# raymondfdavey/Conditioned-Diffusion-Models-UAD

Measured on AMD Instinct MI355X. Metric: reconstructed 128x128 slices/sec @ T=1000, higher is better.
Workload: dtype f32_emulated_f16x3

## Files before the change

conditioned-diffusion-models-uad_amd/_lib.py:

```python
from __future__ import annotations

import ctypes as C
import os

_HERE = os.path.dirname(os.path.abspath(__file__))
LIB_PATH = os.environ.get("CDDPM_LIB") or os.path.join(_HERE, "csrc", "libcddpm_hip.so")

CDDPM_MAX_LEVELS = 8


class UnetDesc(C.Structure):
    _fields_ = [
        ("in_channels", C.c_int32),
        ("out_channels", C.c_int32),
        ("model_channels", C.c_int32),
        ("num_levels", C.c_int32),
        ("channel_mult", C.c_int32 * CDDPM_MAX_LEVELS),
        ("num_res_blocks", C.c_int32),
        ("num_attention_resolutions", C.c_int32),
        ("attention_resolutions", C.c_int32 * CDDPM_MAX_LEVELS),
        ("head_channels", C.c_int32),
        ("cond_dim", C.c_int32),
        ("timesteps", C.c_int32),
        ("max_batch", C.c_int32),
# ... 42 lines not shown
    "cddpm_get_attention_family": (_i, [_vp]),
    "cddpm_set_precision": (_i, [_vp, _i]),
    "cddpm_get_precision": (_i, [_vp]),
    "cddpm_slice_status": (_i, [_vp, _fp, _i, _i, _i, _fp, _vp]),
    "cddpm_set_profiling": (_i, [_vp, _i]),
    "cddpm_get_profile": (_i, [_vp, _i, C.POINTER(C.c_double), C.POINTER(C.c_double), C.POINTER(C.c_double),
                               C.POINTER(_i64)]),
    "cddpm_num_blocks": (_i, [_vp]),
    "cddpm_block_name": (C.c_char_p, [_vp, _i]),
    "cddpm_set_tap": (_i, [_vp, _i, _fp]),
    "cddpm_block_shape": (_i, [_vp, _i, _i, _i, C.POINTER(_i), C.POINTER(_i), C.POINTER(_i)]),
    "cddpm_op_conv": (_i, [_vp, _fp, _i, _fp, _i, _fp, _i, _i, _fp, _fp, _i, _i, _fp, _i, _fp, _i, _i, _i, _vp]),
    "cddpm_op_conv_skip": (_i, [_vp, _fp, _i, _fp, _i, _fp, _fp, _i, _fp, _i, _fp, _fp, _i, _i, _i, _vp]),
    "cddpm_op_conv_gn": (_i, [_vp, _fp, _i, _fp, _fp, _i, _fp, _fp, _fp, _fp, _i, _i, _i, _vp]),
    "cddpm_op_gn_coef": (_i, [_vp, _fp, _i, _fp, _i, _fp, _fp, _fp, _fp, _i, _i, _vp]),
    "cddpm_op_attention": (_i, [_vp, _fp, _fp, _i, _i, _i, _vp]),
    "cddpm_op_attention_p16": (_i, [_vp, _fp, _fp, _i, _i, _i, _vp]),
    "cddpm_op_attention_h3": (_i, [_vp, _fp, _fp, _i, _i, _i, _vp]),
    "cddpm_encoder_create": (_i, [C.POINTER(_vp), _i, _i, _i, _i, _i]),
    "cddpm_encoder_destroy": (None, [_vp]),
    "cddpm_encoder_last_error": (C.c_char_p, [_vp]),
    "cddpm_encoder_num_weights": (_i, []),
    "cddpm_encoder_load_weights": (_i, [_vp, C.POINTER(C.c_char_p), C.POINTER(_fp), C.POINTER(_i64), _i]),
    "cddpm_encoder_forward": (_i, [_vp, _fp, _fp, _i, _i, _i, _vp]),
    "cddpm_op_conv_dgrad": (_i, [_vp, _fp, _i, _fp, _i, _i, _fp, _i, _i, _i, _vp]),
    "cddpm_op_conv_wgrad": (_i, [_vp, _fp, _i, _fp, _i, _fp, _i, _i, _fp, _i, _i, _fp, _fp, _i, _i, _i, _vp]),
    "cddpm_op_bias_grad": (_i, [_vp, _fp, _i64, _i, _fp, _vp]),
    "cddpm_op_attention_backward": (_i, [_vp, _fp, _fp, _fp, _i, _i, _i, _vp]),
    "cddpm_op_attention_backward_p16": (_i, [_vp, _fp, _fp, _fp, _i, _i, _i, _vp]),
    "cddpm_op_attention_backward_h3": (_i, [_vp, _fp, _fp, _fp, _i, _i, _i, _vp]),
    "cddpm_op_linear_backward": (_i, [_vp, _fp, _fp, _fp, _i, _i, _i, _i, _fp, _fp, _fp, _vp]),
    "cddpm_op_linear": (_i, [_vp, _fp, _fp, _fp, _i, _i, _i, _i, _fp, _vp]),
    "cddpm_op_conv_in1": (_i, [_vp, _fp, _fp, _fp, _fp, _i, _i, _i, _i, _vp]),
    "cddpm_op_head": (_i, [_vp, _fp, _fp, _fp, C.c_float, _fp, _fp, _i, _i, _i, _i, _vp]),
    "cddpm_op_pool_act": (_i, [_vp, _fp, _fp, _fp, _fp, _i, _i, _i, _i, _vp]),
    "cddpm_op_unpool2": (_i, [_vp, _fp, _fp, _i, _i, _i, _i, C.c_float, _i, _vp]),
    "cddpm_op_sumpool2": (_i, [_vp, _fp, _fp, _i, _i, _i, _i, _i, _vp]),
    "cddpm_op_add_inplace": (_i, [_vp, _fp, _fp, _i64, _vp]),
    "cddpm_op_act_dropout": (_i, [_vp, _fp, _fp, _i, _fp, _u64, _u32, _u64, _u32, C.c_double, _i, _i, _i, _vp]),
    "cddpm_op_dropout_scale": (_i, [_vp, _fp, _u64, _u32, _u64, _u32, C.c_double, _i, _i, _i, _vp]),
    "cddpm_op_chan_image_corr": (_i, [_vp, _fp, _fp, _i, _fp, _i, _fp, _i, _i, _i, _i, _vp]),
    "cddpm_op_head_dgrad": (_i, [_vp, _fp, _fp, _fp, _i, _i, _i, _i, _vp]),
    "cddpm_op_loss": (_i, [_vp, _fp, _fp, _fp, _i, _i, _i, C.c_float, _fp, _fp, _vp]),
    "cddpm_op_loss_box": (_i, [_vp, _fp, _fp, _fp, _vp, _fp, _i, _i, _i, _i, _i, _i, C.c_float, _vp, _fp, _fp, _vp]),
    "cddpm_box_q_sample": (_i, [_vp, _fp, _fp, _vp, _i, _fp, _fp, _i, _vp, _fp, _i, _i, _i, _i, _vp]),
    "cddpm_box_stitch": (_i, [_vp, _fp, _vp, _vp, _i, _fp, _i, _i, _i, _i, _vp]),
    "cddpm_op_adam": (_i, [_vp, _fp, _fp, _fp, _fp, _i64, C.c_float, C.c_float, C.c_float, C.c_float, _i, C.c_float, _vp]),
    "cddpm_set_train_precision": (_i, [_i]),
    "cddpm_get_train_precision": (_i, []),
    "cddpm_op_grad_check": (_i, [_vp, _fp, _i64, _vp, _vp]),
    "cddpm_op_guard_commit": (_i, [_vp, _vp, C.c_float, C.c_float, _vp]),
    "cddpm_op_adam_guarded": (_i, [_vp, _fp, _fp, _fp, _fp, _i64, C.c_float, C.c_float, C.c_float, C.c_float, C.c_float, _vp, _vp]),
    "cddpm_op_loss_scaled": (_i, [_vp, _fp, _fp, _fp, _i, _i, _i, _vp, _fp, _fp, _vp]),
    "cddpm_op_adam_scaled": (_i, [_vp, _fp, _fp, _fp, _fp, _i64, C.c_float, C.c_float, C.c_float, C.c_float, C.c_float, _vp, _vp, _vp]),
    "cddpm_op_scaler_update": (_i, [_vp, _vp, _vp, C.c_float, C.c_float, _i, _vp]),
    "cddpm_op_gn_silu_backward": (_i, [_vp, _fp, _fp, _i, _fp, _fp, _fp, _fp, _i, _fp, _fp, _fp, _fp, _fp, _fp, _i, _fp, _i, _i, _i, _vp]),
    "cddpm_op_enc_pack_w": (_i, [_vp, _fp, _i, _i, _i, _fp, _fp, _vp]),
    "cddpm_op_enc_conv": (_i, [_vp, _fp, _fp, _fp, _i, _i, _i, _i, _i, _i, _i, _i, _vp]),
    "cddpm_op_enc_conv_wgrad": (_i, [_vp, _fp, _fp, _fp, _i, _i, _i, _i, _i, _i, _i, _vp]),
    "cddpm_op_enc_pack_w_p16": (_i, [_vp, _fp, _i, _i, _i, _vp, _vp, _vp]),
    "cddpm_op_enc_conv_p16": (_i, [_vp, _fp, _vp, _fp, _i, _i, _i, _i, _i, _i, _i, _i, _vp]),
    "cddpm_op_enc_conv_wgrad_p16": (_i, [_vp, _fp, _fp, _fp, _i, _i, _i, _i, _i, _i, _i, _vp]),
    "cddpm_op_enc_stem": (_i, [_vp, _fp, _fp, _fp, _i, _i, _i, _vp]),
    "cddpm_op_enc_stem_wgrad": (_i, [_vp, _fp, _fp, _fp, _i, _i, _i, _vp]),
    "cddpm_op_enc_bn_forward": (_i, [_vp, _fp, _fp, _fp, _fp, _fp, _i, C.c_float, C.c_float, _fp, _fp, _fp, _fp, _i64, _i, _i, _vp]),
    "cddpm_op_enc_bn_backward": (_i, [_vp, _fp, _fp, _fp, _fp, _fp, _fp, _i, _fp, _fp, _fp, _fp, _i64, _i, _i, _vp]),
# ... 88 lines not shown
```

conditioned-diffusion-models-uad_amd/csrc/cddpm_api.hip:

```cpp
#include "cddpm_ctx.h"

#include <cmath>
#include <cstdarg>
#include <cstdio>
#include <cstdlib>

using namespace cddpm;

namespace {
thread_local std::string g_create_error;
}

int cddpm::fail(cddpm_ctx* h, const char* fmt, ...) {
    char buf[1024];
    va_list ap;
    va_start(ap, fmt);
    vsnprintf(buf, sizeof buf, fmt, ap);
    va_end(ap);
    if (h) h->err = buf; else g_create_error = buf;
    return -1;
}

namespace {

// ... 252 lines not shown
        if (op.kind != OP_HEAD) maxact = std::max(maxact, elems);
        if (op.push) {
            float* p = nullptr;
            want(&p, elems);
            h->hs.push_back(p);
        }
    }
    for (const ResW& r : h->res) maxC = std::max(maxC, (size_t)std::max(r.Cin, r.Cout));
    for (const AttnW& a : h->attn) maxC = std::max(maxC, (size_t)a.C);
    want(&h->bufA, maxact);
    want(&h->bufB, maxact);
    want(&h->bufH, maxact);
    want(&h->bufP0, maxact / 4 + 16);
    want(&h->bufP1, maxact / 4 + 16);
    size_t maxqkv = 0, maxatt = 0;
    for (const Op& op : h->prog)
        if (op.kind == OP_ATTN) {
            const BlockInfo& bi = h->blocks[op.block];
            const AttnW& a = h->attn[op.idx];
            int dsa = bi.ds;
            for (const Op& o2 : h->prog)
                if (o2.block == op.block && o2.kind == OP_RES && h->res[o2.idx].up) dsa = bi.ds * 2;
            const size_t n = HW / ((size_t)dsa * dsa);
            maxqkv = std::max(maxqkv, B * n * 3 * a.C);
            maxatt = std::max(maxatt, B * n * a.C);
        }
    want(&h->qkvbuf, maxqkv);
    want(&h->attbuf, maxatt);
    want(&h->headP, B * HW * 9);
    want(&h->model_out, B * HW);
    {
        auto nrec_at = [&](int ds) {
            const int hh = d.max_h / ds, ww = d.max_w / ds;
            return std::max(std::max(conv_stat_records(hh, ww), conv_stat_records_up2(hh, ww)), gn_nsplit(1, hh * ww));
        };
        size_t pi = 0;
        for (const Op& op : h->prog)
            if (op.push) {
                const BlockInfo& bi = h->blocks[op.block];
                const size_t cap = B * (size_t)nrec_at(bi.ds) * bi.C * 2;
                float* sp = nullptr;
                want(&sp, cap);
                if (do_alloc) h->stat[h->hs[pi]] = {sp, cap, STAT_NONE};
                ++pi;
            }
        size_t maxrc = 0;
        for (const BlockInfo& bi : h->blocks) maxrc = std::max(maxrc, (size_t)nrec_at(bi.ds) * bi.C);
        float* work[3] = {h->bufA, h->bufB, h->bufH};
        for (int i = 0; i < 3; ++i) {
            float* sp = nullptr;
            want(&sp, B * maxrc * 2);
            if (do_alloc) h->stat[work[i]] = {sp, B * maxrc * 2, STAT_NONE};
        }
    }
    want(&h->coef, 3 * B * maxC);
    want(&h->kpart, (size_t)KSPLIT_PLANE_FLOATS);
    const size_t rows = std::max<size_t>(d.timesteps, B);
    want(&h->tab, (size_t)d.timesteps * h->sumE);
    want(&h->cpart, B * (size_t)h->sumE);
    want(&h->scratch0, rows * std::max(h->half, d.model_channels));
    want(&h->scratch1, rows * h->half);
    for (int i = 0; i < 5; ++i) want(&h->sched[i], d.timesteps);
    want(&h->qs_sa, d.timesteps);
    want(&h->qs_s1, d.timesteps);
    total += B * sizeof(int);
    if (do_alloc && *rc == 0) *rc = dev_alloc(h, &h->d_t, B);
    for (const WeightSpec& w : h->wspecs) total += (size_t)w.numel * sizeof(float);
// ... 140 lines not shown
        return fail(h, "H=%d W=%d invalid for this handle (multiples of %d, max %dx%d)", H, W, q > 4 ? q : 4, h->d.max_h, h->d.max_w);
    if (h->cond_B != B) return fail(h, "cddpm_prepare_cond was last called for B=%d, this call has B=%d", h->cond_B, B);
    return 0;
}

int stage_t(cddpm_ctx* h, const int32_t* t_dev, int t_uniform, int B, hipStream_t s) {
    if (t_dev) {
        launch_copy_clamp_int(h->d_t, t_dev, B, 0, h->d.timesteps - 1, s);
    } else {
        if (t_uniform < 0 || t_uniform >= h->d.timesteps) return fail(h, "t=%d outside [0, %d)", t_uniform, h->d.timesteps);
        launch_fill_int(h->d_t, B, t_uniform, s);
    }
    return 0;
}

int forward_impl(cddpm_ctx* h, const float* x, float* out, int B, int H, int W, hipStream_t s) {
    for (auto& kv : h->stat) kv.second.valid_count = STAT_NONE;
    h->cur_H = H; h->cur_W = W;
    std::vector<int> stack;
    int npush = 0;
    const float* cur = nullptr;
    int curC = 0, curds = 1;
    float* pp[2] = {h->bufA, h->bufB};
    int ppi = 0;
    for (size_t oi = 0; oi < h->prog.size(); ++oi) {
        const Op& op = h->prog[oi];
        const BlockInfo& bi = h->blocks[op.block];
        float* dst;
        if (op.push) dst = h->hs[npush];
        else { dst = pp[ppi]; ppi ^= 1; }
        const int Hc = H / curds, Wc = W / curds;
        switch (op.kind) {
            case OP_IN: {
                Prof pi(h, PC_OTHER, 18.0 * B * H * W * h->d.model_channels, 4.0 * B * (double)H * W * (h->d.model_channels + 1), s);
                launch_conv_in1(x, h->in_w, h->in_b, dst, B, H, W, h->d.model_channels, s);
            }
                curC = h->d.model_channels;
                break;
            case OP_RES: {
                const ResW& r = h->res[op.idx];
                const float* x1 = nullptr;
                int C1 = 0;
                if (op.concat) {
                    const int si = stack.back();
                    stack.pop_back();
                    x1 = h->hs[si];
                    C1 = r.Cin - curC;
                }
                if (dst == cur) { dst = pp[ppi]; ppi ^= 1; }
                if (run_res(h, r, cur, curC, x1, C1, dst, B, Hc, Wc, s)) return -1;
                curC = r.Cout;
                if (r.down) curds *= 2;
                if (r.up) curds /= 2;
                break;
            }
            case OP_ATTN:
                if (dst == cur) { dst = pp[ppi]; ppi ^= 1; }
                if (run_attn(h, h->attn[op.idx], cur, dst, B, Hc, Wc, s)) return -1;
                break;
            case OP_HEAD: {
                if (gn_coef(h, cur, curC, nullptr, 0, B, H * W, h->out_norm, false, 0, s)) return -1;
                Prof ph(h, PC_OTHER, 18.0 * B * H * W * curC, 4.0 * B * (double)H * W * (curC + 19), s);
                launch_head_dots(cur, h->coef, h->head_w9, h->headP, B, H * W, curC, s);
                launch_head_gather(h->headP, h->head_bias, nullptr, out, B, H, W, s);
                dst = nullptr;
                break;
            }
        }
// ... 722 lines not shown
```

conditioned-diffusion-models-uad_amd/csrc/cddpm_ops.hip:

```cpp
#include "cddpm_ctx.h"

#include <cmath>

using namespace cddpm;

template <class Request> static size_t counted(Request&& request) {
    OpScratch sc;
    request(sc);
    return sc.off;
}

extern "C" {

int cddpm_op_set_scratch(cddpm_handle h, size_t bytes) {
    if (!h) return -1;
    HIPCHECK(h, hipSetDevice(h->device));
    HIPCHECK(h, hipDeviceSynchronize());
    if (h->arena) { (void)hipFree(h->arena); h->arena = nullptr; h->arena_bytes = 0; }
    if (bytes) { HIPCHECK(h, hipMalloc(&h->arena, bytes)); h->arena_bytes = bytes; }
    return 0;
}

static int need_zero_bias(cddpm_ctx* h) {
    if (h->zero_bias) return 0;
// ... 292 lines not shown
    OP_EPILOGUE()
}

static float* linear_backward_scratch(OpScratch& sc, int M, int N, int K, int silu_in) {
    const size_t nscr = linear_backward_scratch_floats(M, N, K, silu_in);
    return nscr ? sc.n<float>(nscr) : nullptr;
}
size_t cddpm_op_linear_backward_scratch(int M, int N, int K, int silu_in) {
    return counted([&](OpScratch& sc) { linear_backward_scratch(sc, M, N, K, silu_in); });
}
int cddpm_op_linear_backward(cddpm_handle h, const float* x_dev, const float* w_dev, const float* dy_dev, int M, int N, int K,
                             int silu_in, float* dw_dev, float* db_dev, float* dx_dev, void* stream) {
    OP_PROLOGUE(PC_OTHER, 0.0, 0.0, M >= 1 && N >= 1 && K >= 1 && x_dev && w_dev && dy_dev && dw_dev, "cddpm_op_linear_backward: bad arguments")
    OpScratch sc(h, s);
    float* a = linear_backward_scratch(sc, M, N, K, silu_in);
    SCRATCH_CHECK(sc)
    launch_linear_backward(x_dev, w_dev, dy_dev, M, N, K, silu_in, a, dw_dev, db_dev, dx_dev, s);
    OP_EPILOGUE()
}

int cddpm_op_linear(cddpm_handle h, const float* x_dev, const float* w_dev, const float* b_dev, int M, int N, int K, int silu_in,
                    float* y_dev, void* stream) {
    OP_CHECK(M >= 1 && N >= 1 && K >= 1 && K % 4 == 0, "cddpm_op_linear: unsupported shape (M %d, N %d, K %d: all >= 1, K a multiple of 4)", M, N, K)
    OP_PROLOGUE(PC_OTHER, 0.0, 0.0, x_dev && w_dev && y_dev && !(((uintptr_t)x_dev | (uintptr_t)w_dev) & 15),
                "cddpm_op_linear: NULL argument, or x_dev / w_dev not 16-byte aligned")
    launch_linear(x_dev, K, w_dev, K, 0, b_dev, y_dev, N, M, N, K, silu_in, s);
    OP_EPILOGUE()
}
int cddpm_op_conv_in1(cddpm_handle h, const float* x_dev, const float* w_dev, const float* b_dev, float* out_dev, int B, int H, int W,
                      int C, void* stream) {
    OP_CHECK(B >= 1 && H >= 1 && W >= 1 && (long long)B * H * W < (1ll << 31) && C >= 64 && C % 64 == 0 && C <= 512,
             "cddpm_op_conv_in1: unsupported shape (B %d, H %d, W %d: all >= 1, B * H * W < 2^31; C %d: a multiple of 64, at most 512)", B, H, W, C)
    OP_PROLOGUE(PC_OTHER, 0.0, 0.0, x_dev && w_dev && b_dev && out_dev, "cddpm_op_conv_in1: NULL argument")
    launch_conv_in1(x_dev, w_dev, b_dev, out_dev, B, H, W, C, s);
    OP_EPILOGUE()
}
static float* head_scratch(OpScratch& sc, int B, int H, int W) { return sc.n<float>((size_t)B * H * W * 9); }
size_t cddpm_op_head_scratch(int B, int H, int W, int) { return counted([&](OpScratch& sc) { head_scratch(sc, B, H, W); }); }
int cddpm_op_head(cddpm_handle h, const float* x_dev, const float* coef_dev, const float* w9_dev, float bias, const float* bias_dev,
                  float* out_dev, int B, int H, int W, int C, void* stream) {
    static_assert(head_dots_lds_bytes(head_max_channels()) <= LDS_BYTES_PER_WORKGROUP && head_dots_lds_bytes(head_max_channels() + 32) > LDS_BYTES_PER_WORKGROUP,
                  "the widest head");
    OP_CHECK(B >= 1 && H >= 1 && W >= 1 && C >= 32 && C % 32 == 0 && C <= head_max_channels(),
             "cddpm_op_head: unsupported shape (B %d, H %d, W %d: all >= 1; C %d: a multiple of 32, at most %d)", B, H, W, C, head_max_channels())
    OP_PROLOGUE(PC_OTHER, 0.0, 0.0, x_dev && coef_dev && w9_dev && out_dev, "cddpm_op_head: NULL argument")
    OpScratch sc(h, s);
    float* P = head_scratch(sc, B, H, W);
    SCRATCH_CHECK(sc)
    launch_head_dots(x_dev, coef_dev, w9_dev, P, B, H * W, C, s);
    launch_head_gather(P, bias, bias_dev, out_dev, B, H, W, s);
    OP_EPILOGUE()
}
static bool resample_shape_ok(int B, int H, int W, int C) { return B >= 1 && H >= 2 && W >= 2 && H % 2 == 0 && W % 2 == 0 && C >= 4 && C % 4 == 0; }
int cddpm_op_pool_act(cddpm_handle h, const float* x_dev, const float* coef_dev, float* hp_dev, float* xp_dev, int B, int H, int W, int C,
                      void* stream) {
    OP_CHECK(resample_shape_ok(B, H, W, C), "cddpm_op_pool_act: unsupported shape (B %d >= 1; H %d, W %d: even, >= 2; C %d: a multiple of 4, >= 4)", B, H, W, C)
    OP_PROLOGUE(PC_OTHER, 0.0, 0.0, x_dev && coef_dev && hp_dev && xp_dev, "cddpm_op_pool_act: NULL argument")
    launch_pool_act(x_dev, coef_dev, hp_dev, xp_dev, B, H, W, C, s);
    OP_EPILOGUE()
}
int cddpm_op_unpool2(cddpm_handle h, const float* dyp_dev, float* dx_dev, int B, int H, int W, int C, float scale, int accumulate, void* stream) {
    OP_CHECK(resample_shape_ok(B, H, W, C), "cddpm_op_unpool2: unsupported shape (B %d >= 1; H %d, W %d: even, >= 2; C %d: a multiple of 4, >= 4)", B, H, W, C)
    OP_PROLOGUE(PC_OTHER, 0.0, 0.0, dyp_dev && dx_dev, "cddpm_op_unpool2: NULL argument")
    launch_unpool2(dyp_dev, dx_dev, B, H, W, C, scale, accumulate, s);
    OP_EPILOGUE()
}
int cddpm_op_sumpool2(cddpm_handle h, const float* dy_dev, float* dxp_dev, int B, int H, int W, int C, int accumulate, void* stream) {
// ... 600 lines not shown
```

conditioned-diffusion-models-uad_amd/csrc/conv_split.h:

```cpp
#pragma once
#include <hip/hip_runtime.h>

namespace cddpm {

typedef float f32x16 __attribute__((ext_vector_type(16)));
typedef float v4f __attribute__((ext_vector_type(4)));
typedef float v2f __attribute__((ext_vector_type(2)));
typedef __bf16 bf16x8 __attribute__((ext_vector_type(8)));
typedef __bf16 bf16x4 __attribute__((ext_vector_type(4)));
typedef _Float16 f16x8 __attribute__((ext_vector_type(8)));
typedef _Float16 f16x4 __attribute__((ext_vector_type(4)));

template <int NS> struct SplitT;
template <> struct SplitT<3> {
    typedef bf16x8 v8; typedef bf16x4 v4;
    static __device__ __forceinline__ f32x16 mfma(v8 a, v8 b, f32x16 c) { return __builtin_amdgcn_mfma_f32_32x32x16_bf16(a, b, c, 0, 0, 0); }
};
template <> struct SplitT<2> {
    typedef f16x8 v8; typedef f16x4 v4;
    static __device__ __forceinline__ f32x16 mfma(v8 a, v8 b, f32x16 c) { return __builtin_amdgcn_mfma_f32_32x32x16_f16(a, b, c, 0, 0, 0); }
};

__device__ __forceinline__ float silu_x6(float v) {
    const float t = fminf(-v * 1.44269502162933349609375f, 126.0f);
    float tl = __builtin_fmaf(-v, 1.44269502162933349609375f, -t);
    tl = __builtin_fmaf(-v, 1.925963033500011e-08f, tl);
    tl = (t < 126.0f) ? tl : 0.0f;
    float e = __builtin_amdgcn_exp2f(t);
    e = __builtin_fmaf(e, tl * 0.693147180559945f, e);
    return v * __builtin_amdgcn_rcpf(1.0f + e);
}

__device__ __forceinline__ v4f silu_x6_v4(const v4f v) {
    const v4f nl2e = {-1.44269502162933349609375f, -1.44269502162933349609375f, -1.44269502162933349609375f, -1.44269502162933349609375f};
    const v4f nl2e_lo = {-1.925963033500011e-08f, -1.925963033500011e-08f, -1.925963033500011e-08f, -1.925963033500011e-08f};
    const v4f lim = {126.0f, 126.0f, 126.0f, 126.0f};
    const v4f ln2 = {0.693147180559945f, 0.693147180559945f, 0.693147180559945f, 0.693147180559945f};
    const v4f one = {1.0f, 1.0f, 1.0f, 1.0f};
    const v4f t = __builtin_elementwise_min(v * nl2e, lim);
    v4f tl = __builtin_elementwise_fma(v, nl2e, -t);
    tl = __builtin_elementwise_fma(v, nl2e_lo, tl);
    v4f e = {__builtin_amdgcn_exp2f(t.x), __builtin_amdgcn_exp2f(t.y), __builtin_amdgcn_exp2f(t.z), __builtin_amdgcn_exp2f(t.w)};
    e = __builtin_elementwise_fma(e, tl * ln2, e);
    const v4f d = one + e;
    const v4f r = {__builtin_amdgcn_rcpf(d.x), __builtin_amdgcn_rcpf(d.y), __builtin_amdgcn_rcpf(d.z), __builtin_amdgcn_rcpf(d.w)};
    return v * r;
}

template <int NS>
__device__ __forceinline__ void split_x4(const v4f v, typename SplitT<NS>::v4 (&t)[NS]) {
    typedef typename SplitT<NS>::v4 q4;
    v4f r = v;
#pragma unroll
    for (int s = 0; s < NS; ++s) {
        t[s] = __builtin_convertvector(r, q4);
        r = r - __builtin_convertvector(t[s], v4f);
    }
}

}
```

conditioned-diffusion-models-uad_amd/csrc/conv_x6.hip:

```cpp
#include "kernels.h"
#include "conv_split.h"
#include <algorithm>
#include <cstdlib>
#include <cstring>
#include <type_traits>
#include <vector>

namespace cddpm {

static constexpr int ROWS = 8;
template <int TAPS, int NS, bool HI1 = false, int NB = 1>
__global__ __launch_bounds__(64 * ROWS) void conv_split_kernel(const ConvArgs a) {
    static_assert(NB == 1 || (NB == 2 && NS == 2 && TAPS != 1), "two cout blocks per workgroup: 16 x 16 fp16 form, LDS-DMA loop (3x3 and folded 2x2) only");
    typedef typename SplitT<NS>::v8 frag;
    constexpr int SP = 4 * NS;
    constexpr int THREADS = 64 * ROWS;
    constexpr bool UP2 = (TAPS == 4);
    constexpr int PAD = (TAPS == 9) ? 1 : 0;
    constexpr int PW = UP2 ? 33 : 32 + 2 * PAD;
    constexpr int PH = UP2 ? ROWS + 1 : ROWS + 2 * PAD;
    constexpr int NPIX = PW * PH;
    constexpr int NK = (NPIX * 8 + THREADS - 1) / THREADS;
    constexpr int FOLD = (TAPS == 9) ? 3 : (TAPS == 4 ? 2 : 1);
    constexpr int WSLOTS = 128 * SP;
// ... 78 lines not shown
    const bool have_coef = (a.coef != nullptr);

    auto wslab = [&](int chunk, int tap) -> const v4f* {
        if (chunk >= nch) { chunk = 0; tap = 0; }
        return (chunk < nch_main) ? (wmain + ((size_t)chunk * TAPS + tap) * WSLOTS)
                                  : (wskip + (size_t)(chunk - nch_main) * WSLOTS);
    };
    auto load_act = [&](int chunk) {
        const float* base;
        int Cs, c0;
        const bool main_seg = chunk < nch_main;
        if (main_seg) {
            const int ch = chunk << 5;
            if (ch < a.C0) { base = a.src0; Cs = a.C0; c0 = ch; }
            else           { base = a.src1; Cs = a.C1; c0 = ch - a.C0; }
        } else {
            const int ch = (chunk - nch_main) << 5;
            if (ch < a.S0) { base = a.skip0; Cs = a.S0; c0 = ch; }
            else           { base = a.skip1; Cs = a.S1; c0 = ch - a.S0; }
        }
        const float* ubase = base + ((size_t)b * a.srcH * a.srcW * Cs + c0);
#pragma unroll
        for (int k = 0; k < NK; ++k) {
            const int p = (main_seg || ((centre >> k) & 1u)) ? psrc[k] : -1;
            v4f v = v4f{0.f, 0.f, 0.f, 0.f};
            if (p >= 0) v = *reinterpret_cast<const v4f*>(ubase + (__umul24((unsigned)p, (unsigned)Cs) + 4u * (unsigned)c4));
            areg[k] = v;
        }
    };
    typename SplitT<NS>::v4 sreg[NK][NS];
    auto transform_act = [&](int chunk) {
        const bool main_seg = chunk < nch_main;
        const bool do_silu = main_seg && a.silu;
        v4f cm = v4f{0.f, 0.f, 0.f, 0.f}, ca = v4f{1.f, 1.f, 1.f, 1.f}, cd = cm;
        const bool aff = main_seg && have_coef;
        if (aff) {
            const int ci = (chunk << 3) + c4;
            cm = ldsC[ci];
            ca = ldsC[(Cin >> 2) + ci];
            cd = ldsC[2 * (Cin >> 2) + ci];
        }
#pragma unroll
        for (int k = 0; k < NK; ++k) {
            v4f v = areg[k];
            const int p = (main_seg || ((centre >> k) & 1u)) ? psrc[k] : -1;
            if (p >= 0) {
                v = (v - cm) * ca + cd;
                if (do_silu) {
                    if constexpr (NS == 2) v = silu_x6_v4(v);
                    else { v.x = silu_x6(v.x); v.y = silu_x6(v.y); v.z = silu_x6(v.z); v.w = silu_x6(v.w); }
                }
            }
            split_x4<NS>(v, sreg[k]);
        }
    };
    auto write_act = [&]() {
        v2f* dst = reinterpret_cast<v2f*>(ldsA);
#pragma unroll
        for (int k = 0; k < NK; ++k) {
            const int q = (tid >> 3) + (THREADS / 8) * k;
            if (q < NPIX) {
#pragma unroll
                for (int sp = 0; sp < (HI1 ? 1 : NS); ++sp) {
                    const int sl = M16 ? (q * 8 + ((4 * sp + (c4 >> 1)) ^ (int)((colswz >> (3 * k)) & 7u))) : slot_a(q, sp, c4 >> 1);
                    dst[sl * 2 + (c4 & 1)] = __builtin_bit_cast(v2f, sreg[k][sp]);
                }
            }
        }
    };
    auto store_act = [&](int chunk) { transform_act(chunk); write_act(); };

    typedef float f32x4 __attribute__((ext_vector_type(4)));
    f32x16 acc[2][2], tot[2][2];
    f32x4 acc16[NB][4][4], tot16[4][4];
    if constexpr (M16) {
#pragma unroll
        for (int i = 0; i < 4; ++i)
#pragma unroll
            for (int j = 0; j < 4; ++j) {
                tot16[i][j] = f32x4{0.f, 0.f, 0.f, 0.f};
// ... 568 lines not shown
```

conditioned-diffusion-models-uad_amd/csrc/kernels.h:

```cpp
#pragma once
#include <hip/hip_runtime.h>
#include <stdint.h>

namespace cddpm {

#define CDDPM_MAX_KSPLIT 8
struct ConvArgs {
    const float* src0;
    const float* src1;
    int C0, C1;
    int srcH, srcW;
    int upsample;
    const float* coef;
    int silu;
    const float* wpk;
    const float* bias;
    const float* res;
    int res_up;
    float* out;
    int B, H, W, Cout;
    int taps;
    const float* skip0; const float* skip1; int S0, S1;
    const float* skip_wpk;
    float* stats;
// ... 2 lines not shown
    short kbound[CDDPM_MAX_KSPLIT + 1];
    int hi_only;
    int nb2;
    int family;
};
bool conv_nb2_ok(int Cout, long long workgroups128, int ksplit, int family);
int conv_nb2_env();
void launch_conv_reduce(const float* planes, int ksplit, const float* bias, const float* res, int res_up, float* out, float* stats,
                        int B, int H, int W, int Cout, hipStream_t stream);
inline int conv_reduce_stat_records(int H, int W) { return (H * W + 63) / 64; }
#define CDDPM_STAT_FLOATS 2
inline int conv_stat_records(int H, int W) { return 2 * ((W + 31) / 32) * ((H + 3) / 4); }
inline int conv_stat_records_up2(int H, int W) { return 8 * ((W / 2 + 31) / 32) * ((H / 2 + 3) / 4); }
void launch_conv(const ConvArgs& a, hipStream_t stream);
int conv_mode();
void launch_conv_split(const ConvArgs& a, hipStream_t stream);
int conv_weight_exp(const float* w, size_t n, int family);
void pack_conv_weights_split(const float* w , int Cout, int Cin, int taps, void* dst, int wexp, int family);

size_t packed_conv_floats(int Cout, int Cin, int taps, int family);
void launch_pack_conv_split(const float* w_dev, int O, int I, int taps, int mode, int wexp, void* dst_dev, hipStream_t stream);
struct PackJob { const float* w; void* dst; int O, I, taps, mode, wexp, cls; };
void launch_pack_conv_split_batch(const PackJob* jobs_dev, int njobs, long long max_units, hipStream_t stream);
void launch_absmax(const float* x, long long n, float* out, hipStream_t stream);
void pack_conv_weights(const float* w , int Cout, int Cin, int taps, float* dst, int wexp, int family);
int pack_conv_weights_up2(const float* w , int Cout, int Cin, float* dst, int family);

void launch_gn_partial(const float* src, int C, int B, int HW, int nsplit, float* rec, hipStream_t stream);
int gn_nsplit(int B, int HW);
void launch_gn_finalize(const float* rec0, int C0, int n0, const float* rec1, int C1, int n1, int B, int HW,
                        const float* gamma, const float* beta, const float* tab, const float* cpart, int sumE, int eoff,
                        const int* t_dev, const float* film_direct, float* coef, hipStream_t stream);

void launch_conv_in1(const float* x, const float* w, const float* bias, float* out, int B, int H, int W, int C,
                     hipStream_t stream);
constexpr size_t LDS_BYTES_PER_WORKGROUP = 160 * 1024;
constexpr size_t head_dots_lds_bytes(int C) { return ((size_t)64 * (C + 4) + (size_t)9 * C) * sizeof(float); }
constexpr int head_max_channels() {
    int C = 32;
    while (head_dots_lds_bytes(C + 32) <= LDS_BYTES_PER_WORKGROUP) C += 32;
    return C;
}
void launch_head_dots(const float* x, const float* coef, const float* w9 , float* P, int B, int HW, int C,
                      hipStream_t stream);
void launch_head_gather(const float* P, float bias, const float* bias_ptr , float* out, int B, int H, int W,
                        hipStream_t stream);
void launch_pool_act(const float* x, const float* coef, float* hp, float* xp, int B, int H, int W, int C,
                     hipStream_t stream);
void launch_linear(const float* x, int ldx, const float* W, int ldw, int koff, const float* bias, float* y, int ldy,
                   int M, int N, int K, int silu_in, hipStream_t stream);
void launch_fill_int(int* p, int n, int v, hipStream_t stream);
void launch_add_int(int* p, int n, int v, hipStream_t stream);
void launch_copy_clamp_int(int* dst, const int* src, int n, int lo, int hi, hipStream_t stream);
void launch_slice_status(const float* x, int B, int HW, int* status, hipStream_t stream);

struct StepArgs {
    float* x; const float* model_out; const int* t_dev;
    const float* coef1; const float* coef2; const float* logvar; const float* sqrt_recip; const float* sqrt_recipm1;
    int objective;
    const float* noise;
    size_t noise_t_stride;
    uint64_t seed, slice0; int t_for_rng;
    int B, HW;
    int finalize;
    int clip;
};
void launch_step(const StepArgs& a, hipStream_t stream);
// ... 171 lines not shown
```

conditioned-diffusion-models-uad_amd/csrc/small_kernels.hip:

```cpp
#include "kernels.h"

namespace cddpm {

__device__ __forceinline__ float silu_s(float v) {
    const float t = fminf(-v * 1.44269502162933349609375f, 126.0f);
    float tl = __builtin_fmaf(-v, 1.44269502162933349609375f, -t);
    tl = __builtin_fmaf(-v, 1.925963033500011e-08f, tl);
    tl = (t < 126.0f) ? tl : 0.0f;
    float e = __builtin_amdgcn_exp2f(t);
    e = __builtin_fmaf(e, tl * 0.693147180559945f, e);
    return v * __builtin_amdgcn_rcpf(1.0f + e);
}

__global__ __launch_bounds__(256) void conv_in1_kernel(const float* __restrict__ x, const float* __restrict__ w,
                                                       const float* __restrict__ bias, float* __restrict__ out,
                                                       int B, int H, int W, int C) {
    const int ncq = C >> 2, npl = 256 / ncq;
    const int tid = threadIdx.x;
    const int cq = tid % ncq, pl = tid / ncq;
    float wr[4][9], br[4];
#pragma unroll
    for (int i = 0; i < 4; ++i) {
        br[i] = bias[4 * cq + i];
#pragma unroll
        for (int t = 0; t < 9; ++t) wr[i][t] = w[(4 * cq + i) * 9 + t];
    }
    const unsigned total = (unsigned)B * H * W;
    const unsigned ppb = 16u * npl;
    const unsigned pend = min(total, (blockIdx.x + 1u) * ppb);
    for (unsigned p = blockIdx.x * ppb + pl; p < pend; p += npl) {
        const unsigned row = p / (unsigned)W;
        const int xx = (int)(p - row * W);
        const unsigned bb = row / (unsigned)H;
        const int yy = (int)(row - bb * H);
        const float* img = x + (size_t)bb * H * W;
        float v[9];
#pragma unroll
        for (int ky = 0; ky < 3; ++ky)
#pragma unroll
            for (int kx = 0; kx < 3; ++kx) {
                const int y2 = yy + ky - 1, x2 = xx + kx - 1;
                v[ky * 3 + kx] = (y2 >= 0 && y2 < H && x2 >= 0 && x2 < W) ? img[y2 * W + x2] : 0.f;
            }
        float4 o;
        float* op = &o.x;
#pragma unroll
        for (int i = 0; i < 4; ++i) {
            float acc = br[i];
#pragma unroll
            for (int t = 0; t < 9; ++t) acc = fmaf(v[t], wr[i][t], acc);
            op[i] = acc;
        }
        *reinterpret_cast<float4*>(out + (size_t)p * C + 4 * cq) = o;
    }
}

void launch_conv_in1(const float* x, const float* w, const float* bias, float* out, int B, int H, int W, int C,
                     hipStream_t stream) {
    const int npl = 256 / (C / 4);
    const long long total = (long long)B * H * W;
    const int ppb = 16 * npl;
    hipLaunchKernelGGL(conv_in1_kernel, dim3((unsigned)((total + ppb - 1) / ppb)), dim3(256), 0, stream, x, w, bias, out,
                       B, H, W, C);
}

__global__ __launch_bounds__(256) void head_dots_kernel(const float* __restrict__ x, const float* __restrict__ coef,
                                                        const float* __restrict__ w9, float* __restrict__ P, int B,
                                                        int HW, int C) {
    extern __shared__ float hl[];
    float* lx = hl;
    float* lw = hl + 64 * (C + 4);
    const int tid = threadIdx.x;
    const long long total = (long long)B * HW;
    const long long pix0 = (long long)blockIdx.x * 64;
    const int ncq = C >> 2;
    const size_t plane = (size_t)B * C;
    for (int i = tid; i < 9 * C; i += 256) lw[i] = w9[i];
    for (int e = tid; e < 64 * ncq; e += 256) {
        const int pl = e / ncq, cq = e - pl * ncq;
        const long long p = pix0 + pl;
        float4 v = make_float4(0.f, 0.f, 0.f, 0.f);
        if (p < total) {
            const int b = (int)(p / HW);
            v = *reinterpret_cast<const float4*>(x + p * C + 4 * cq);
            const size_t ci = (size_t)b * C + 4 * cq;
            const float4 m = *reinterpret_cast<const float4*>(coef + ci);
            const float4 a = *reinterpret_cast<const float4*>(coef + plane + ci);
            const float4 d = *reinterpret_cast<const float4*>(coef + 2 * plane + ci);
            v.x = silu_s((v.x - m.x) * a.x + d.x);
            v.y = silu_s((v.y - m.y) * a.y + d.y);
            v.z = silu_s((v.z - m.z) * a.z + d.z);
            v.w = silu_s((v.w - m.w) * a.w + d.w);
        }
        *reinterpret_cast<float4*>(lx + pl * (C + 4) + 4 * cq) = v;
    }
    __syncthreads();
// ... 505 lines not shown
```

include/cddpm.h:

```cpp
#ifndef CDDPM_H
#define CDDPM_H

#include <stddef.h>
#include <stdint.h>

#ifdef __cplusplus
extern "C" {
#endif

typedef struct cddpm_ctx* cddpm_handle;

#define CDDPM_MAX_LEVELS 8

typedef struct cddpm_unet_desc {
    int32_t in_channels;
    int32_t out_channels;
    int32_t model_channels;
    int32_t num_levels;
    int32_t channel_mult[CDDPM_MAX_LEVELS];
    int32_t num_res_blocks;
    int32_t num_attention_resolutions;
    int32_t attention_resolutions[CDDPM_MAX_LEVELS];
    int32_t head_channels;
    int32_t cond_dim;
// ... 223 lines not shown
int cddpm_op_conv_skip(cddpm_handle h, const float* src0_dev, int C0, const float* coef_dev, int silu,
                       const float* w_host, const float* bias_host, int Cout, const float* skip_dev, int S0,
                       const float* wskip_host, float* out_dev, int B, int H, int W, void* stream);

int cddpm_op_conv_gn(cddpm_handle h, const float* src0_dev, int C0, const float* w_host, const float* bias_host, int Cout,
                     const float* gamma_host, const float* beta_host, float* out_dev, float* coef_dev, int B, int H, int W,
                     void* stream);

int cddpm_op_gn_coef(cddpm_handle h, const float* src0_dev, int C0, const float* src1_dev, int C1,
                     const float* gamma_host, const float* beta_host, const float* film_dev,
                     float* coef_dev, int B, int HW, void* stream);

size_t cddpm_packed_conv_bytes(int Cout, int Cin, int taps);
int cddpm_pack_conv_weights(const float* w_host, int Cout, int Cin, int taps, void* dst_host, int* scale_exp_out);

int cddpm_op_conv_dgrad(cddpm_handle h, const float* dy_dev, int Cout, const float* w_host, int Cin, int ksize, float* dx_dev,
                        int B, int H, int W, void* stream);
int cddpm_op_conv_wgrad(cddpm_handle h, const float* x0_dev, int C0, const float* x1_dev, int C1, const float* coef_dev, int silu,
                        int upsample, const float* dy_dev, int Cout, int ksize, float* dw_dev, float* db_dev, int B, int H, int W,
                        void* stream);
int cddpm_op_bias_grad(cddpm_handle h, const float* dy_dev, int64_t npix, int C, float* db_dev, void* stream);
int cddpm_op_attention_backward(cddpm_handle h, const float* qkv_dev, const float* da_dev, float* dqkv_dev, int B, int N, int C,
                                void* stream);
int cddpm_op_attention_backward_p16(cddpm_handle h, const float* qkv_dev, const float* da_dev, float* dqkv_dev, int B, int N, int C,
                                    void* stream);
int cddpm_op_attention_backward_h3(cddpm_handle h, const float* qkv_dev, const float* da_dev, float* dqkv_dev, int B, int N, int C,
                                   void* stream);
int cddpm_op_linear_backward(cddpm_handle h, const float* x_dev, const float* w_dev, const float* dy_dev, int M, int N, int K,
                             int silu_in, float* dw_dev, float* db_dev, float* dx_dev, void* stream);
int cddpm_op_linear(cddpm_handle h, const float* x_dev, const float* w_dev, const float* b_dev, int M, int N, int K, int silu_in,
                    float* y_dev, void* stream);
int cddpm_op_conv_in1(cddpm_handle h, const float* x_dev, const float* w_dev, const float* b_dev, float* out_dev, int B, int H, int W,
                      int C, void* stream);
int cddpm_op_head(cddpm_handle h, const float* x_dev, const float* coef_dev, const float* w9_dev, float bias, const float* bias_dev,
                  float* out_dev, int B, int H, int W, int C, void* stream);
int cddpm_op_pool_act(cddpm_handle h, const float* x_dev, const float* coef_dev, float* hp_dev, float* xp_dev, int B, int H, int W, int C,
                      void* stream);
int cddpm_op_unpool2(cddpm_handle h, const float* dyp_dev, float* dx_dev, int B, int H, int W, int C, float scale, int accumulate, void* stream);
int cddpm_op_sumpool2(cddpm_handle h, const float* dy_dev, float* dxp_dev, int B, int H, int W, int C, int accumulate, void* stream);
int cddpm_op_add_inplace(cddpm_handle h, float* a_dev, const float* b_dev, int64_t n, void* stream);
int cddpm_op_act_dropout(cddpm_handle h, const float* x_dev, const float* coef_dev, int silu, float* out_dev, uint64_t seed, uint32_t step,
                         uint64_t slice0, uint32_t stream_id, double p, int B, int HW, int C, void* stream);
int cddpm_op_dropout_scale(cddpm_handle h, float* da_dev, uint64_t seed, uint32_t step, uint64_t slice0, uint32_t stream_id, double p, int B,
                           int HW, int C, void* stream);
int cddpm_op_chan_image_corr(cddpm_handle h, const float* t_dev, const float* coef_dev, int silu, const float* s_dev, int sign, float* dw_dev,
                             int B, int H, int W, int C, void* stream);
int cddpm_op_head_dgrad(cddpm_handle h, const float* dout_dev, const float* w9_dev, float* dact_dev, int B, int H, int W, int C, void* stream);
int cddpm_op_loss(cddpm_handle h, const float* out_dev, const float* target_dev, const float* w_b_dev, int l2, int B, int HW, float grad_scale,
                  float* dout_dev, float* loss_b_dev, void* stream);
int cddpm_op_loss_box(cddpm_handle h, const float* out_dev, const float* x0_dev, const float* noise_dev, const int32_t* box_dev,
                      const float* w_b_dev, int pred_noise, int inpaint, int l2, int B, int H, int W, float grad_scale,
                      const int32_t* scaler_dev, float* dout_dev, float* loss_b_dev, void* stream);
int cddpm_op_adam(cddpm_handle h, float* p_dev, const float* g_dev, float* m_dev, float* v_dev, int64_t n, float lr, float beta1, float beta2,
                  float eps, int step, float grad_unscale, void* stream);
int cddpm_set_train_precision(int bits);
int cddpm_get_train_precision(void);
int cddpm_op_grad_check(cddpm_handle h, const float* g_dev, int64_t n, int32_t* ctrl_dev, void* stream);
int cddpm_op_guard_commit(cddpm_handle h, int32_t* ctrl_dev, float beta1, float beta2, void* stream);
int cddpm_op_adam_guarded(cddpm_handle h, float* p_dev, const float* g_dev, float* m_dev, float* v_dev, int64_t n, float lr, float beta1,
                          float beta2, float eps, float grad_unscale, const int32_t* ctrl_dev, void* stream);
int cddpm_op_loss_scaled(cddpm_handle h, const float* out_dev, const float* target_dev, const float* w_b_dev, int l2, int B, int HW,
                         const int32_t* scaler_dev, float* dout_dev, float* loss_b_dev, void* stream);
int cddpm_op_adam_scaled(cddpm_handle h, float* p_dev, const float* g_dev, float* m_dev, float* v_dev, int64_t n, float lr, float beta1,
                         float beta2, float eps, float extra_unscale, const int32_t* ctrl_dev, const int32_t* scaler_dev, void* stream);
int cddpm_op_scaler_update(cddpm_handle h, const int32_t* ctrl_dev, int32_t* scaler_dev, float growth, float backoff, int interval,
                           void* stream);
// ... 104 lines not shown
```

Measured before the change: 1.431.

## Fuse GroupNorm statistics into input convolution and tighten f16 split and SiLU

The input 3x3 convolution now accumulates per-block, per-channel sums and sums of squares in double and writes GroupNorm statistic records. The following GroupNorm can reuse these records instead of reading the full activation again to compute them. The grid is reorganised to one run of blocks per image so records line up with the per-image layout, and the stat buffer capacity check is extended to cover them. It also adds a v_fma_mix based split_x4<2> specialisation and rearranges the SiLU and affine arithmetic in the conv kernel to save a few instructions, at the cost of double-precision reductions and a shared-memory pass in the input conv.

```diff
diff --git a/conditioned-diffusion-models-uad_amd/_lib.py b/conditioned-diffusion-models-uad_amd/_lib.py
--- a/conditioned-diffusion-models-uad_amd/_lib.py
+++ b/conditioned-diffusion-models-uad_amd/_lib.py
@@ -98,6 +98,8 @@
     "cddpm_op_linear_backward": (_i, [_vp, _fp, _fp, _fp, _i, _i, _i, _i, _fp, _fp, _fp, _vp]),
     "cddpm_op_linear": (_i, [_vp, _fp, _fp, _fp, _i, _i, _i, _i, _fp, _vp]),
     "cddpm_op_conv_in1": (_i, [_vp, _fp, _fp, _fp, _fp, _i, _i, _i, _i, _vp]),
+    "cddpm_conv_in1_records": (_i, [_i, _i, _i]),
+    "cddpm_op_conv_in1_stats": (_i, [_vp, _fp, _fp, _fp, _fp, _fp, _i, _i, _i, _i, _vp]),
     "cddpm_op_head": (_i, [_vp, _fp, _fp, _fp, C.c_float, _fp, _fp, _i, _i, _i, _i, _vp]),
     "cddpm_op_pool_act": (_i, [_vp, _fp, _fp, _fp, _fp, _i, _i, _i, _i, _vp]),
     "cddpm_op_unpool2": (_i, [_vp, _fp, _fp, _i, _i, _i, _i, C.c_float, _i, _vp]),
diff --git a/conditioned-diffusion-models-uad_amd/csrc/cddpm_api.hip b/conditioned-diffusion-models-uad_amd/csrc/cddpm_api.hip
--- a/conditioned-diffusion-models-uad_amd/csrc/cddpm_api.hip
+++ b/conditioned-diffusion-models-uad_amd/csrc/cddpm_api.hip
@@ -308,7 +308,8 @@
     {
         auto nrec_at = [&](int ds) {
             const int hh = d.max_h / ds, ww = d.max_w / ds;
-            return std::max(std::max(conv_stat_records(hh, ww), conv_stat_records_up2(hh, ww)), gn_nsplit(1, hh * ww));
+            const int n = std::max(std::max(conv_stat_records(hh, ww), conv_stat_records_up2(hh, ww)), gn_nsplit(1, hh * ww));
+            return ds == 1 ? std::max(n, conv_in1_records(hh * ww, d.model_channels)) : n;
         };
         size_t pi = 0;
         for (const Op& op : h->prog)
@@ -515,8 +516,15 @@
         const int Hc = H / curds, Wc = W / curds;
         switch (op.kind) {
             case OP_IN: {
-                Prof pi(h, PC_OTHER, 18.0 * B * H * W * h->d.model_channels, 4.0 * B * (double)H * W * (h->d.model_channels + 1), s);
-                launch_conv_in1(x, h->in_w, h->in_b, dst, B, H, W, h->d.model_channels, s);
+                const int Cm = h->d.model_channels, nrec = conv_in1_records(H * W, Cm);
+                StatBuf& sb = h->stat.at(dst);
+                const size_t need = (size_t)B * nrec * Cm * 2;
+                if (need > sb.capacity)
+                    return fail(h, "GroupNorm statistics records of the %dx%dx%d input convolution (B=%d, %d records) need %zu floats, the buffer holds %zu",
+                                H, W, Cm, B, nrec, need, sb.capacity);
+                Prof pi(h, PC_OTHER, 18.0 * B * H * W * Cm, 4.0 * B * (double)H * W * (Cm + 1), s);
+                launch_conv_in1(x, h->in_w, h->in_b, dst, sb.records, B, H, W, Cm, s);
+                sb.valid_count = nrec;
             }
                 curC = h->d.model_channels;
                 break;
diff --git a/conditioned-diffusion-models-uad_amd/csrc/cddpm_ops.hip b/conditioned-diffusion-models-uad_amd/csrc/cddpm_ops.hip
--- a/conditioned-diffusion-models-uad_amd/csrc/cddpm_ops.hip
+++ b/conditioned-diffusion-models-uad_amd/csrc/cddpm_ops.hip
@@ -348,7 +348,20 @@
     OP_CHECK(B >= 1 && H >= 1 && W >= 1 && (long long)B * H * W < (1ll << 31) && C >= 64 && C % 64 == 0 && C <= 512,
              "cddpm_op_conv_in1: unsupported shape (B %d, H %d, W %d: all >= 1, B * H * W < 2^31; C %d: a multiple of 64, at most 512)", B, H, W, C)
     OP_PROLOGUE(PC_OTHER, 0.0, 0.0, x_dev && w_dev && b_dev && out_dev, "cddpm_op_conv_in1: NULL argument")
-    launch_conv_in1(x_dev, w_dev, b_dev, out_dev, B, H, W, C, s);
+    launch_conv_in1(x_dev, w_dev, b_dev, out_dev, nullptr, B, H, W, C, s);
+    OP_EPILOGUE()
+}
+int cddpm_conv_in1_records(int H, int W, int C) {
+    if (H < 1 || W < 1 || (long long)H * W >= (1ll << 31) || C < 64 || C % 64 || C > 512) return -1;
+    return conv_in1_records(H * W, C);
+}
+int cddpm_op_conv_in1_stats(cddpm_handle h, const float* x_dev, const float* w_dev, const float* b_dev, float* out_dev, float* rec_dev, int B,
+                            int H, int W, int C, void* stream) {
+    OP_CHECK(B >= 1 && H >= 1 && W >= 1 && (long long)B * H * W < (1ll << 31) && C >= 64 && C % 64 == 0 && C <= 512,
+             "cddpm_op_conv_in1_stats: unsupported shape (B %d, H %d, W %d: all >= 1, B * H * W < 2^31; C %d: a multiple of 64, at most 512)", B, H, W, C)
+    OP_PROLOGUE(PC_OTHER, 0.0, 0.0, x_dev && w_dev && b_dev && out_dev && rec_dev && !((uintptr_t)rec_dev & 15),
+                "cddpm_op_conv_in1_stats: NULL argument, or rec_dev not 16-byte aligned")
+    launch_conv_in1(x_dev, w_dev, b_dev, out_dev, rec_dev, B, H, W, C, s);
     OP_EPILOGUE()
 }
 static float* head_scratch(OpScratch& sc, int B, int H, int W) { return sc.n<float>((size_t)B * H * W * 9); }
diff --git a/conditioned-diffusion-models-uad_amd/csrc/conv_split.h b/conditioned-diffusion-models-uad_amd/csrc/conv_split.h
--- a/conditioned-diffusion-models-uad_amd/csrc/conv_split.h
+++ b/conditioned-diffusion-models-uad_amd/csrc/conv_split.h
@@ -32,15 +32,16 @@
 }
 
 __device__ __forceinline__ v4f silu_x6_v4(const v4f v) {
+    const v4f l2e = {1.44269502162933349609375f, 1.44269502162933349609375f, 1.44269502162933349609375f, 1.44269502162933349609375f};
     const v4f nl2e = {-1.44269502162933349609375f, -1.44269502162933349609375f, -1.44269502162933349609375f, -1.44269502162933349609375f};
     const v4f nl2e_lo = {-1.925963033500011e-08f, -1.925963033500011e-08f, -1.925963033500011e-08f, -1.925963033500011e-08f};
-    const v4f lim = {126.0f, 126.0f, 126.0f, 126.0f};
+    const v4f nlim = {-126.0f, -126.0f, -126.0f, -126.0f};
     const v4f ln2 = {0.693147180559945f, 0.693147180559945f, 0.693147180559945f, 0.693147180559945f};
     const v4f one = {1.0f, 1.0f, 1.0f, 1.0f};
-    const v4f t = __builtin_elementwise_min(v * nl2e, lim);
-    v4f tl = __builtin_elementwise_fma(v, nl2e, -t);
+    const v4f nt = __builtin_elementwise_max(v * l2e, nlim);
+    v4f tl = __builtin_elementwise_fma(v, nl2e, nt);
     tl = __builtin_elementwise_fma(v, nl2e_lo, tl);
-    v4f e = {__builtin_amdgcn_exp2f(t.x), __builtin_amdgcn_exp2f(t.y), __builtin_amdgcn_exp2f(t.z), __builtin_amdgcn_exp2f(t.w)};
+    v4f e = {__builtin_amdgcn_exp2f(-nt.x), __builtin_amdgcn_exp2f(-nt.y), __builtin_amdgcn_exp2f(-nt.z), __builtin_amdgcn_exp2f(-nt.w)};
     e = __builtin_elementwise_fma(e, tl * ln2, e);
     const v4f d = one + e;
     const v4f r = {__builtin_amdgcn_rcpf(d.x), __builtin_amdgcn_rcpf(d.y), __builtin_amdgcn_rcpf(d.z), __builtin_amdgcn_rcpf(d.w)};
@@ -58,4 +59,18 @@
     }
 }
 
+template <>
+__device__ __forceinline__ void split_x4<2>(const v4f v, f16x4 (&t)[2]) {
+    typedef unsigned u32x2 __attribute__((ext_vector_type(2)));
+    t[0] = __builtin_convertvector(v, f16x4);
+    const u32x2 hp = __builtin_bit_cast(u32x2, t[0]);
+    const float m1 = -1.0f;
+    v4f r;
+    asm("v_fma_mix_f32 %0, %1, %2, %3 op_sel_hi:[1,0,0]" : "=v"(r.x) : "v"(hp.x), "s"(m1), "v"(v.x));
+    asm("v_fma_mix_f32 %0, %1, %2, %3 op_sel:[1,0,0] op_sel_hi:[1,0,0]" : "=v"(r.y) : "v"(hp.x), "s"(m1), "v"(v.y));
+    asm("v_fma_mix_f32 %0, %1, %2, %3 op_sel_hi:[1,0,0]" : "=v"(r.z) : "v"(hp.y), "s"(m1), "v"(v.z));
+    asm("v_fma_mix_f32 %0, %1, %2, %3 op_sel:[1,0,0] op_sel_hi:[1,0,0]" : "=v"(r.w) : "v"(hp.y), "s"(m1), "v"(v.w));
+    t[1] = __builtin_convertvector(r, f16x4);
 }
+
+}
diff --git a/conditioned-diffusion-models-uad_amd/csrc/conv_x6.hip b/conditioned-diffusion-models-uad_amd/csrc/conv_x6.hip
--- a/conditioned-diffusion-models-uad_amd/csrc/conv_x6.hip
+++ b/conditioned-diffusion-models-uad_amd/csrc/conv_x6.hip
@@ -134,11 +134,11 @@
     auto transform_act = [&](int chunk) {
         const bool main_seg = chunk < nch_main;
         const bool do_silu = main_seg && a.silu;
-        v4f cm = v4f{0.f, 0.f, 0.f, 0.f}, ca = v4f{1.f, 1.f, 1.f, 1.f}, cd = cm;
+        v4f ncm = v4f{-0.f, -0.f, -0.f, -0.f}, ca = v4f{1.f, 1.f, 1.f, 1.f}, cd = v4f{0.f, 0.f, 0.f, 0.f};
         const bool aff = main_seg && have_coef;
         if (aff) {
             const int ci = (chunk << 3) + c4;
-            cm = ldsC[ci];
+            ncm = -ldsC[ci];
             ca = ldsC[(Cin >> 2) + ci];
             cd = ldsC[2 * (Cin >> 2) + ci];
         }
@@ -147,7 +147,7 @@
             v4f v = areg[k];
             const int p = (main_seg || ((centre >> k) & 1u)) ? psrc[k] : -1;
             if (p >= 0) {
-                v = (v - cm) * ca + cd;
+                v = (v + ncm) * ca + cd;
                 if (do_silu) {
                     if constexpr (NS == 2) v = silu_x6_v4(v);
                     else { v.x = silu_x6(v.x); v.y = silu_x6(v.y); v.z = silu_x6(v.z); v.w = silu_x6(v.w); }
diff --git a/conditioned-diffusion-models-uad_amd/csrc/kernels.h b/conditioned-diffusion-models-uad_amd/csrc/kernels.h
--- a/conditioned-diffusion-models-uad_amd/csrc/kernels.h
+++ b/conditioned-diffusion-models-uad_amd/csrc/kernels.h
@@ -58,7 +58,8 @@
                         const float* gamma, const float* beta, const float* tab, const float* cpart, int sumE, int eoff,
                         const int* t_dev, const float* film_direct, float* coef, hipStream_t stream);
 
-void launch_conv_in1(const float* x, const float* w, const float* bias, float* out, int B, int H, int W, int C,
+int conv_in1_records(int HW, int C);
+void launch_conv_in1(const float* x, const float* w, const float* bias, float* out, float* rec, int B, int H, int W, int C,
                      hipStream_t stream);
 constexpr size_t LDS_BYTES_PER_WORKGROUP = 160 * 1024;
 constexpr size_t head_dots_lds_bytes(int C) { return ((size_t)64 * (C + 4) + (size_t)9 * C) * sizeof(float); }
diff --git a/conditioned-diffusion-models-uad_amd/csrc/small_kernels.hip b/conditioned-diffusion-models-uad_amd/csrc/small_kernels.hip
--- a/conditioned-diffusion-models-uad_amd/csrc/small_kernels.hip
+++ b/conditioned-diffusion-models-uad_amd/csrc/small_kernels.hip
@@ -12,12 +12,19 @@
     return v * __builtin_amdgcn_rcpf(1.0f + e);
 }
 
+constexpr int CONV_IN1_PIXELS_PER_LANE = 16;
+int conv_in1_records(int HW, int C) {
+    const int ppb = CONV_IN1_PIXELS_PER_LANE * (256 / (C / 4));
+    return (HW + ppb - 1) / ppb;
+}
+template <bool STATS>
 __global__ __launch_bounds__(256) void conv_in1_kernel(const float* __restrict__ x, const float* __restrict__ w,
                                                        const float* __restrict__ bias, float* __restrict__ out,
-                                                       int B, int H, int W, int C) {
+                                                       float* __restrict__ rec, int nrun, int H, int W, int C) {
     const int ncq = C >> 2, npl = 256 / ncq;
     const int tid = threadIdx.x;
     const int cq = tid % ncq, pl = tid / ncq;
+    const int b = blockIdx.x / (unsigned)nrun, run = blockIdx.x - b * nrun;
     float wr[4][9], br[4];
 #pragma unroll
     for (int i = 0; i < 4; ++i) {
@@ -25,43 +32,66 @@
 #pragma unroll
         for (int t = 0; t < 9; ++t) wr[i][t] = w[(4 * cq + i) * 9 + t];
     }
-    const unsigned total = (unsigned)B * H * W;
-    const unsigned ppb = 16u * npl;
-    const unsigned pend = min(total, (blockIdx.x + 1u) * ppb);
-    for (unsigned p = blockIdx.x * ppb + pl; p < pend; p += npl) {
-        const unsigned row = p / (unsigned)W;
-        const int xx = (int)(p - row * W);
-        const unsigned bb = row / (unsigned)H;
-        const int yy = (int)(row - bb * H);
-        const float* img = x + (size_t)bb * H * W;
-        float v[9];
-#pragma unroll
-        for (int ky = 0; ky < 3; ++ky)
-#pragma unroll
-            for (int kx = 0; kx < 3; ++kx) {
-                const int y2 = yy + ky - 1, x2 = xx + kx - 1;
-                v[ky * 3 + kx] = (y2 >= 0 && y2 < H && x2 >= 0 && x2 < W) ? img[y2 * W + x2] : 0.f;
+    const int HW = H * W;
+    const int ppb = CONV_IN1_PIXELS_PER_LANE * npl;
+    const int p0 = run * ppb;
+    const int pend = min(HW, p0 + ppb);
+    const float* img = x + (size_t)b * HW;
+    float* obase = out + (size_t)b * HW * C + 4 * cq;
+    double s[4] = {0, 0, 0, 0}, q[4] = {0, 0, 0, 0};
+    if (pl < npl) {
+        for (int p = p0 + pl; p < pend; p += npl) {
+            const int yy = (int)((unsigned)p / (unsigned)W);
+            const int xx = p - yy * W;
+            float v[9];
+#pragma unroll
+            for (int ky = 0; ky < 3; ++ky)
+#pragma unroll
+                for (int kx = 0; kx < 3; ++kx) {
+                    const int y2 = yy + ky - 1, x2 = xx + kx - 1;
+                    v[ky * 3 + kx] = (y2 >= 0 && y2 < H && x2 >= 0 && x2 < W) ? img[y2 * W + x2] : 0.f;
+                }
+            float4 o;
+            float* op = &o.x;
+#pragma unroll
+            for (int i = 0; i < 4; ++i) {
+                float acc = br[i];
+#pragma unroll
+                for (int t = 0; t < 9; ++t) acc = fmaf(v[t], wr[i][t], acc);
+                op[i] = acc;
+                if constexpr (STATS) {
+                    const double d = (double)acc;
+                    s[i] += d;
+                    q[i] = fma(d, d, q[i]);
+                }
             }
-        float4 o;
-        float* op = &o.x;
-#pragma unroll
-        for (int i = 0; i < 4; ++i) {
-            float acc = br[i];
-#pragma unroll
-            for (int t = 0; t < 9; ++t) acc = fmaf(v[t], wr[i][t], acc);
-            op[i] = acc;
-        }
-        *reinterpret_cast<float4*>(out + (size_t)p * C + 4 * cq) = o;
-    }
-}
-
-void launch_conv_in1(const float* x, const float* w, const float* bias, float* out, int B, int H, int W, int C,
+            *reinterpret_cast<float4*>(obase + (size_t)p * C) = o;
+        }
+    }
+    if constexpr (STATS) {
+        __shared__ double red[256][9];
+#pragma unroll
+        for (int i = 0; i < 4; ++i) { red[tid][i] = s[i]; red[tid][4 + i] = q[i]; }
+        __syncthreads();
+        if (tid < ncq) {
+            double ts[4] = {0, 0, 0, 0}, tq[4] = {0, 0, 0, 0};
+            for (int l = 0; l < npl; ++l) {
+#pragma unroll
+                for (int i = 0; i < 4; ++i) { ts[i] += red[l * ncq + tid][i]; tq[i] += red[l * ncq + tid][4 + i]; }
+            }
+            float* o = rec + ((size_t)blockIdx.x * C + 4 * tid) * 2;
+            *reinterpret_cast<float4*>(o) = make_float4((float)ts[0], (float)tq[0], (float)ts[1], (float)tq[1]);
+            *reinterpret_cast<float4*>(o + 4) = make_float4((float)ts[2], (float)tq[2], (float)ts[3], (float)tq[3]);
+        }
+    }
+}
+
+void launch_conv_in1(const float* x, const float* w, const float* bias, float* out, float* rec, int B, int H, int W, int C,
                      hipStream_t stream) {
-    const int npl = 256 / (C / 4);
-    const long long total = (long long)B * H * W;
-    const int ppb = 16 * npl;
-    hipLaunchKernelGGL(conv_in1_kernel, dim3((unsigned)((total + ppb - 1) / ppb)), dim3(256), 0, stream, x, w, bias, out,
-                       B, H, W, C);
+    const int nrun = conv_in1_records(H * W, C);
+    const dim3 grid((unsigned)B * (unsigned)nrun);
+    if (rec) hipLaunchKernelGGL(conv_in1_kernel<true>, grid, dim3(256), 0, stream, x, w, bias, out, rec, nrun, H, W, C);
+    else hipLaunchKernelGGL(conv_in1_kernel<false>, grid, dim3(256), 0, stream, x, w, bias, out, rec, nrun, H, W, C);
 }
 
 __global__ __launch_bounds__(256) void head_dots_kernel(const float* __restrict__ x, const float* __restrict__ coef,
diff --git a/include/cddpm.h b/include/cddpm.h
--- a/include/cddpm.h
+++ b/include/cddpm.h
@@ -279,6 +279,9 @@
                     float* y_dev, void* stream);
 int cddpm_op_conv_in1(cddpm_handle h, const float* x_dev, const float* w_dev, const float* b_dev, float* out_dev, int B, int H, int W,
                       int C, void* stream);
+int cddpm_conv_in1_records(int H, int W, int C);
+int cddpm_op_conv_in1_stats(cddpm_handle h, const float* x_dev, const float* w_dev, const float* b_dev, float* out_dev, float* rec_dev, int B,
+                            int H, int W, int C, void* stream);
 int cddpm_op_head(cddpm_handle h, const float* x_dev, const float* coef_dev, const float* w9_dev, float bias, const float* bias_dev,
                   float* out_dev, int B, int H, int W, int C, void* stream);
 int cddpm_op_pool_act(cddpm_handle h, const float* x_dev, const float* coef_dev, float* hp_dev, float* xp_dev, int B, int H, int W, int C,
```

Result: slower. 1.315 (-8.1%).
